# snakers4/mnasnet-pytorch

Hardware: AMD Instinct MI355X
Metric: images/sec MNASNet-1.0 224^2 bf16 train step (higher is better)
Workload: dtype bf16

## Files before the change

include/mnas.h:

```cpp
#ifndef MNAS_H
#define MNAS_H
#include <stdint.h>

#ifdef __cplusplus
extern "C" {
#endif

#define MNAS_OK 0
#define MNAS_EINVAL 10001
#define MNAS_BN_ROWS 8

typedef struct MnasActIn {
    const void*  data;
    const float* scale;
    const float* shift;
} MnasActIn;

typedef struct MnasGradIn {
    const void*  g;
    const void*  y;
    const float* coef;
} MnasGradIn;

int mnas_version(void);
// ... 172 lines not shown
    MnasPostWgrad w1, w2;
} MnasBwdPost;
int mnas_bwd_post(const MnasBwdPost* p, void* stream);

typedef struct MnasBnFrozenDesc {
    const float* gamma;
    const float* beta;
    const float* running_mean;
    const float* running_var;
    float*  bnbuf;
    int32_t C;
    float   eps;
} MnasBnFrozenDesc;
int mnas_bn_frozen_tables(const MnasBnFrozenDesc* descs, int n, void* stream);
int mnas_bn_bwd_finalize_frozen(const float* partial, int nparts, int C, const float* bnbuf, float* dgamma, float* dbeta,
                                float* dbias, int accumulate, void* stream);
typedef struct MnasBwdPostFrozen {
    const float* bn_partial;
    const float* bnbuf;
    float* dgamma;
    float* dbeta;
    double count;
    int32_t bn_nparts, bn_C;
    MnasPostWgrad w1, w2;
    float* dbias;
} MnasBwdPostFrozen;
int mnas_bwd_post_frozen(const MnasBwdPostFrozen* p, void* stream);

int mnas_add_act(const MnasActIn* a, const MnasActIn* b, int64_t rows, int C, void* out_bf16,
                 float* out_nchw_f32, int HW, void* stream);
int mnas_pool_act(const MnasActIn* a, int N, int HW, int C, float* out, void* stream);
int mnas_pool_bwd(const float* gpool, int N, int HW, int C, void* g_bf16, void* stream);
int mnas_nchw_f32_to_nhwc_bf16(const float* src, void* dst, int N, int C, int HW, void* stream);

typedef struct MnasHeadLinear {
    int32_t N, I, O;
    int32_t relu;
    int32_t accumulate;
    float   drop_p;
    uint64_t seed;
    const void* x;
    const void* w;
    const void* b;
    void*       y;
    const void* dz;
    void*       dw;
    void*       db;
    void*       dx;
    const void* relu_mask;
} MnasHeadLinear;
int mnas_head_linear_fwd(const MnasHeadLinear* a, void* stream);
int mnas_head_linear_bwd_w(const MnasHeadLinear* a, void* stream);
int mnas_head_linear_bwd_x(const MnasHeadLinear* a, void* stream);
int mnas_head_dropout_mask(void* out_u8, int64_t n, float p, uint64_t seed, void* stream);
int mnas_head_cross_entropy(const void* logits, const void* target, int N, int C, int64_t ignore_index,
                            void* loss_rows, void* loss, void* dlogits, void* bad_flag, void* stream);

#define MNAS_METERS_MAX_K   4
#define MNAS_METERS_NUM_I64 14
#define MNAS_METERS_NUM_F64 3
typedef struct MnasMeters {
    int64_t steps;
    int64_t samples;
    int64_t loss_samples;
    int64_t nonfinite_steps;
    int64_t correct[MNAS_METERS_MAX_K];
    int64_t last_n;
    int64_t last_loss_n;
    int64_t last_correct[MNAS_METERS_MAX_K];
    double  loss_sum;
    double  last_loss;
    double  last_loss_sum;
} MnasMeters;
int mnas_head_cross_entropy_metrics(const void* logits, const void* target, int N, int C, int64_t ignore_index,
                                    void* loss_rows, void* loss, void* dlogits, void* bad_flag, const int* ks, int nk,
                                    void* rank_rows, MnasMeters* meters, void* stream);
int mnas_head_metrics(const void* logits, const void* target, int N, int C, const int* ks, int nk, const void* loss,
                      void* rank_rows, MnasMeters* meters, void* stream);

int mnas_head_cross_entropy_soft(const void* logits, const void* target_a, const void* target_b, const float* lam,
                                 float label_smoothing, int N, int C, int64_t ignore_index, void* loss_rows, void* loss,
                                 void* dlogits, void* bad_flag, const int* ks, int nk, void* rank_rows, MnasMeters* meters,
                                 void* stream);

#define MNAS_MLABEL_NUM_I64 16
#define MNAS_MLABEL_NUM_F64 9
typedef struct MnasMultiLabelMeters {
    int64_t steps;
    int64_t samples;
    int64_t nonfinite_steps;
    int64_t loss_n;
    int64_t dice_n;
    int64_t f1_n;
    int64_t tp;
    int64_t fp;
    int64_t fn;
    int64_t last_n;
    int64_t last_loss_n;
    int64_t last_dice_n;
    int64_t last_f1_n;
    int64_t last_tp;
    int64_t last_fp;
    int64_t last_fn;
    double  loss_sum;
    double  dice_sum;
    double  f1_sum;
// ... 224 lines not shown
```

mnasnet_pytorch_amd/_lib.py:

```python
from __future__ import annotations

import ctypes as C
import os

import torch

_HERE = os.path.dirname(os.path.abspath(__file__))
ABI_VERSION = 8
LIB_PATH = os.environ.get("MNAS_LIB_PATH") or os.path.join(_HERE, "csrc", "libmnas_hip.so")

c_void_p, c_int, c_float, c_double, c_int64 = C.c_void_p, C.c_int, C.c_float, C.c_double, C.c_int64


class MnasActIn(C.Structure):
    _fields_ = [("data", c_void_p), ("scale", c_void_p), ("shift", c_void_p)]


class MnasGradIn(C.Structure):
    _fields_ = [("g", c_void_p), ("y", c_void_p), ("coef", c_void_p)]


class MnasConvGemm(C.Structure):
    _fields_ = [("mode", C.c_int32), ("N", C.c_int32), ("Hi", C.c_int32), ("Wi", C.c_int32), ("Ci", C.c_int32),
                ("Ho", C.c_int32), ("Wo", C.c_int32), ("Co", C.c_int32), ("kh", C.c_int32), ("kw", C.c_int32),
# ... 236 lines not shown
    kind, k = _SLOT[o.opcode][name]
    return getattr(o, kind)[k]


def op_ints(o):
    return tuple(int(v) for v in o.i[:len(OP_SLOTS[o.opcode][0])])


class MnasHeadLinear(C.Structure):
    _fields_ = [("N", C.c_int32), ("I", C.c_int32), ("O", C.c_int32), ("relu", C.c_int32), ("accumulate", C.c_int32),
                ("drop_p", c_float), ("seed", C.c_uint64), ("x", c_void_p), ("w", c_void_p), ("b", c_void_p),
                ("y", c_void_p), ("dz", c_void_p), ("dw", c_void_p), ("db", c_void_p), ("dx", c_void_p),
                ("relu_mask", c_void_p)]


METERS_MAX_K, METERS_NUM_I64, METERS_NUM_F64 = 4, 14, 3


class MnasMeters(C.Structure):
    _fields_ = [("steps", c_int64), ("samples", c_int64), ("loss_samples", c_int64), ("nonfinite_steps", c_int64),
                ("correct", c_int64 * 4), ("last_n", c_int64), ("last_loss_n", c_int64), ("last_correct", c_int64 * 4),
                ("loss_sum", c_double), ("last_loss", c_double), ("last_loss_sum", c_double)]


MLABEL_NUM_I64, MLABEL_NUM_F64 = 16, 9


class MnasMultiLabelMeters(C.Structure):
    _fields_ = [(n, c_int64) for n in ("steps", "samples", "nonfinite_steps", "loss_n", "dice_n", "f1_n", "tp", "fp", "fn", "last_n",
                                       "last_loss_n", "last_dice_n", "last_f1_n", "last_tp", "last_fp", "last_fn")] + \
               [(n, c_double) for n in ("loss_sum", "dice_sum", "f1_sum", "last_loss", "last_dice", "last_f1", "last_loss_sum",
                                        "last_dice_sum", "last_f1_sum")]


GRADNORM_MAX_PARTS = 1024


class MnasGradStats(C.Structure):
    _fields_ = [("last_norm", c_float), ("last_coef", c_float), ("steps", c_int64), ("clipped_steps", c_int64),
                ("skipped_steps", c_int64)]


class MnasOptExtra(C.Structure):
    _fields_ = [("partial", c_void_p), ("nparts", C.c_int32), ("max_norm", c_float), ("skip_nonfinite", C.c_int32),
                ("ema", c_void_p), ("ema_decay", c_float), ("stats", c_void_p), ("update_stats", C.c_int32)]


SYMBOLS = {
    "mnas_conv_img_parts": (c_int, [c_int] * 11),
    "mnas_stem_parts": (c_int, [c_int, c_int, c_int, c_int, c_int]),
    "mnas_head_linear_fwd": (c_int, [C.POINTER(MnasHeadLinear), c_void_p]),
    "mnas_head_linear_bwd_w": (c_int, [C.POINTER(MnasHeadLinear), c_void_p]),
    "mnas_head_linear_bwd_x": (c_int, [C.POINTER(MnasHeadLinear), c_void_p]),
    "mnas_head_dropout_mask": (c_int, [c_void_p, c_int64, c_float, C.c_uint64, c_void_p]),
    "mnas_head_cross_entropy": (c_int, [c_void_p, c_void_p, c_int, c_int, c_int64, c_void_p, c_void_p, c_void_p, c_void_p,
                                        c_void_p]),
    "mnas_head_cross_entropy_metrics": (c_int, [c_void_p, c_void_p, c_int, c_int, c_int64, c_void_p, c_void_p, c_void_p, c_void_p,
                                                C.POINTER(c_int), c_int, c_void_p, c_void_p, c_void_p]),
    "mnas_head_metrics": (c_int, [c_void_p, c_void_p, c_int, c_int, C.POINTER(c_int), c_int, c_void_p, c_void_p, c_void_p,
                                  c_void_p]),
    "mnas_head_cross_entropy_soft": (c_int, [c_void_p, c_void_p, c_void_p, c_void_p, c_float, c_int, c_int, c_int64, c_void_p,
                                             c_void_p, c_void_p, c_void_p, C.POINTER(c_int), c_int, c_void_p, c_void_p, c_void_p]),
    "mnas_mlabel_scratch_bytes": (c_int64, [c_int]),
    "mnas_mlabel_bce": (c_int, [c_void_p, c_void_p, c_void_p, c_int, c_int, c_int, c_float, c_float, c_void_p, c_void_p, c_void_p,
                                c_void_p, c_int64, c_int64, c_int64, c_void_p]),
    "mnas_mlabel_metrics": (c_int, [c_void_p, c_void_p, c_int, c_int, c_void_p, c_void_p, c_void_p, c_int64, c_int64, c_int64,
                                    c_void_p]),
    "mnas_mlabel_hard_dice": (c_int, [c_void_p, c_void_p, c_int, c_int, c_float, c_int, c_void_p, c_void_p, c_void_p]),
    "mnas_se_scale": (c_int, [C.POINTER(MnasActIn), c_void_p, c_int, c_int, c_int, c_void_p, c_void_p]),
    "mnas_se_bwd_reduce": (c_int, [c_void_p, C.POINTER(MnasActIn), c_void_p, c_int, c_int, c_int, c_void_p, c_void_p, c_void_p]),
    "mnas_se_scratch_bytes": (c_int64, [c_int, c_int, c_int]),
    "mnas_se_bwd_apply": (c_int, [c_void_p, c_void_p, c_void_p, c_int, c_int, c_int, c_void_p, c_void_p, c_void_p, c_void_p, c_void_p]),
    "mnas_se_bwd_apply_cols": (c_int, [c_int, c_int, c_int]),
    "mnas_se_gate": (c_int, [c_void_p, c_int, c_int, c_void_p, c_void_p]),
    "mnas_se_proj_finalize": (c_int, [c_void_p, c_int, c_int, c_int, c_int, c_void_p, c_void_p, c_void_p, c_int, c_void_p, c_void_p]),
    "mnas_stem_dgrad": (c_int, [c_void_p, c_void_p] + [c_int] * 6 + [c_void_p] * 3),
    "mnas_se_fc_supported": (c_int, [c_int, c_int]),
    "mnas_se_fc_fwd": (c_int, [c_void_p] * 5 + [c_int] * 3 + [c_void_p] * 4),
    "mnas_se_fc_bwd": (c_int, [c_void_p] * 5 + [c_int] * 3 + [c_void_p] * 6 + [c_int, c_void_p]),
    "mnas_conv_gemm_gate_ok": (c_int, [c_int, c_int, c_int, c_int]),
    "mnas_graph_create": (c_int, [C.POINTER(MnasOp), c_int, C.POINTER(c_void_p), c_int, C.POINTER(c_void_p), C.POINTER(c_int)]),
    "mnas_graph_launch": (c_int, [c_void_p, c_void_p]),
    "mnas_graph_destroy": (c_int, [c_void_p]),
    "mnas_version": (c_int, []),
    "mnas_arch": (C.c_char_p, []),
    "mnas_workspace_bytes": (c_int64, [c_int, c_int, c_int, c_int]),
    "mnas_conv_gemm": (c_int, [C.POINTER(MnasConvGemm), c_void_p]),
    "mnas_conv_gemm_route": (c_int, [C.POINTER(MnasConvGemm), C.POINTER(c_int)]),
    "mnas_conv_gemm_instance": (c_int, [C.POINTER(MnasConvGemm), C.POINTER(c_int)]),
    "mnas_conv_gemm_tile_pixels": (c_int, [c_int, c_int, c_int]),
    "mnas_conv_gemm_parts": (c_int, [c_int, c_int, c_int, c_int, c_int]),
    "mnas_conv_wgrad": (c_int, [C.POINTER(MnasConvWgrad), c_void_p]),
    "mnas_conv_wgrad_instance": (c_int, [C.POINTER(MnasConvWgrad), C.POINTER(c_int)]),
    "mnas_conv_wgrad_slabs": (c_int, [c_int, c_int, c_int]),
    "mnas_wgrad_finalize": (c_int, [c_void_p, c_int, c_int, c_int, c_int, c_void_p, c_int, c_void_p]),
    "mnas_pw_bwd": (c_int, [C.POINTER(MnasPwBwd), c_void_p]),
    "mnas_pw_bwd_supported": (c_int, [c_int, c_int]),
    "mnas_pw_bwd_forms": (c_int, [c_int, c_int]),
    "mnas_pw_bwd_instance": (c_int, [C.POINTER(MnasPwBwd), C.POINTER(c_int)]),
    "mnas_pw_bwd_tile_pixels": (c_int, [c_int, c_int]),
    "mnas_pw_bwd_slices": (c_int, [c_int, c_int]),
    "mnas_dw_fwd": (c_int, [C.POINTER(MnasDwFwd), c_void_p]),
    "mnas_dw_bwd": (c_int, [C.POINTER(MnasDwBwd), c_void_p]),
    "mnas_dw_rows": (c_int, [c_int, c_int, c_int, c_int, c_int, c_int, c_int]),
    "mnas_dw_geometry": (c_int, [c_int, c_int, c_int, c_int, c_int, c_int, C.POINTER(c_int)]),
    "mnas_dw_wgrad_finalize": (c_int, [c_void_p, c_int, c_int, c_int, c_void_p, c_int, c_void_p]),
# ... 93 lines not shown
```

mnasnet_pytorch_amd/csrc/mnas_elementwise.hip:

```cpp
#include "mnas_common.h"
#ifndef MNAS_FIN_HOIST
#define MNAS_FIN_HOIST 1
#endif

__device__ __forceinline__ double wave_sum_d(double v) {
#pragma unroll
    for (int o = 32; o > 0; o >>= 1) v += __shfl_xor(v, o, 64);
    return v;
}

template <int TPC>
__device__ __forceinline__ void bn_partial_sums(const float* __restrict__ partial, int nparts, int C, int c, double& s1,
                                                double& s2) {
    const int t = threadIdx.x % TPC;
    const float* p1 = partial + (size_t)c * nparts;
    const float* p2 = partial + ((size_t)C + c) * nparts;
    float a1[4] = {0.f, 0.f, 0.f, 0.f}, a2[4] = {0.f, 0.f, 0.f, 0.f};
    for (int p = t; p < nparts; p += 4 * TPC) {
#pragma unroll
        for (int j = 0; j < 4; ++j) {
            const int pj = p + j * TPC;
            const bool ok = pj < nparts;
            a1[j] += ok ? p1[pj] : 0.f;
            a2[j] += ok ? p2[pj] : 0.f;
// ... 565 lines not shown
        } else {
            const int co = i / K, k = i % K;
            const int tap = k / Ci, ci = k % Ci;
            d = grad + ((size_t)co * Ci + ci) * taps + tap;
        }
        if (accumulate) dold = *d;
    }
#endif
    if (i < total) {
        const float* src = partial + i;
        float a[4] = {0.f, 0.f, 0.f, 0.f};
        for (int p = p0 + ty; p < p1; p += 128) {
            float v[16];
#pragma unroll
            for (int j = 0; j < 16; ++j) {
                const int pj = p + 8 * j;
                v[j] = pj < p1 ? src[(size_t)pj * pstride * total] : 0.f;
            }
#pragma unroll
            for (int j = 0; j < 4; ++j) a[j] += (v[j] + v[j + 4]) + (v[j + 8] + v[j + 12]);
        }
        s += (a[0] + a[1]) + (a[2] + a[3]);
    }
    red[ty][tx] = s;
    __syncthreads();
    if (ty == 0 && i < total) {
#pragma unroll
        for (int j = 1; j < 8; ++j) s += red[j][tx];
        if (FOLD) {
            partial[(size_t)p0 * total + i] = s;
            return;
        }
#if MNAS_FIN_HOIST
        *d = dold + s;
#else
        float* d;
        if (DW) {
            const int tap = i / Co, c = i % Co;
            d = grad + (size_t)c * taps + tap;
        } else {
            const int co = i / K, k = i % K;
            const int tap = k / Ci, ci = k % Ci;
            d = grad + ((size_t)co * Ci + ci) * taps + tap;
        }
        *d = (accumulate ? *d : 0.f) + s;
#endif
    }
}
template <bool DW, bool FOLD>
__global__ __launch_bounds__(256) void k_wgrad_finalize(float* __restrict__ partial, int nsplit, int pstride, int Co, int Ci,
                                                         int taps, float* __restrict__ grad, int accumulate) {
    wgrad_finalize_body<DW, FOLD>(partial, nsplit, pstride, Co, Ci, taps, grad, accumulate, blockIdx.x, blockIdx.y);
}

struct PostWg { float* partial; float* grad; int nsplit, Co, Ci, taps, dw, level, nx, ny; };
struct PostArgs {
    const float* bn_partial; float* bnbuf; float* dgamma; float* dbeta; double count;
    int bn_nparts, bn_C, bn_nblk, bn_wide;
    PostWg w1, w2;
};
__device__ __forceinline__ void post_wg(const PostWg& w, int b) {
    const int bx = b % w.nx, by = b / w.nx;
    if (w.level == 2) {
        if (w.dw) wgrad_finalize_body<true, true>(w.partial, w.nsplit, 1, w.Co, w.Ci, w.taps, w.grad, 1, bx, by);
        else wgrad_finalize_body<false, true>(w.partial, w.nsplit, 1, w.Co, w.Ci, w.taps, w.grad, 1, bx, by);
    } else {
        const int ns = w.level == 3 ? (w.nsplit + FIN_SPLITS - 1) / FIN_SPLITS : w.nsplit;
        const int ps = w.level == 3 ? FIN_SPLITS : 1;
        if (w.dw) wgrad_finalize_body<true, false>(w.partial, ns, ps, w.Co, w.Ci, w.taps, w.grad, 1, bx, by);
        else wgrad_finalize_body<false, false>(w.partial, ns, ps, w.Co, w.Ci, w.taps, w.grad, 1, bx, by);
    }
}
__global__ __launch_bounds__(256) void k_bwd_post(PostArgs a) {
    int b = blockIdx.x;
    if (b < a.bn_nblk) {
        if (a.bn_wide) bn_bwd_finalize_body<256>(a.bn_partial, a.bn_nparts, a.bn_C, a.count, a.bnbuf, a.dgamma, a.dbeta, 1, b);
        else bn_bwd_finalize_body<64>(a.bn_partial, a.bn_nparts, a.bn_C, a.count, a.bnbuf, a.dgamma, a.dbeta, 1, b);
        return;
    }
    b -= a.bn_nblk;
    const int n1 = a.w1.level ? a.w1.nx * a.w1.ny : 0;
    if (b < n1) { post_wg(a.w1, b); return; }
    post_wg(a.w2, b - n1);
}
__global__ __launch_bounds__(256) void k_bwd_post_frozen(PostArgs a, float* dbias) {
    int b = blockIdx.x;
    if (b < a.bn_nblk) {
        if (a.bn_wide) bn_bwd_finalize_body<256, true>(a.bn_partial, a.bn_nparts, a.bn_C, a.count, a.bnbuf, a.dgamma, a.dbeta, 1, b, dbias);
        else bn_bwd_finalize_body<64, true>(a.bn_partial, a.bn_nparts, a.bn_C, a.count, a.bnbuf, a.dgamma, a.dbeta, 1, b, dbias);
        return;
    }
    b -= a.bn_nblk;
    const int n1 = a.w1.level ? a.w1.nx * a.w1.ny : 0;
    if (b < n1) { post_wg(a.w1, b); return; }
    post_wg(a.w2, b - n1);
}
static bool post_fill(PostWg* w, const MnasPostWgrad& t) {
    w->level = t.level;
    if (!t.level) { w->nx = w->ny = 0; return true; }
    if (t.level < 1 || t.level > 3 || !t.partial || !t.grad || t.nsplit < 1 || t.Co < 1 || t.Ci < 1 || t.taps < 1) return false;
    if (t.level == 1 && t.nsplit > 2 * FIN_SPLITS) return false;
    w->partial = t.partial; w->grad = t.grad; w->nsplit = t.nsplit; w->Co = t.Co; w->Ci = t.Ci; w->taps = t.taps; w->dw = t.dw;
    const int total = t.dw ? t.Co * t.taps : t.Co * t.Ci * t.taps;
    w->nx = (total + 31) / 32;
    w->ny = t.level == 2 ? (t.nsplit + FIN_SPLITS - 1) / FIN_SPLITS : 1;
    return true;
}
static int post_args(PostArgs* a, const float* bn_partial, const float* bnbuf, float* dgamma, float* dbeta, double count, int bn_nparts,
                     int bn_C, const MnasPostWgrad& w1, const MnasPostWgrad& w2) {
    if (bn_C > 0) {
        if (!bn_partial || !bnbuf || bn_nparts < 1) return -1;
        a->bn_partial = bn_partial; a->bnbuf = const_cast<float*>(bnbuf); a->dgamma = dgamma; a->dbeta = dbeta; a->count = count;
        a->bn_nparts = bn_nparts; a->bn_C = bn_C;
        a->bn_wide = bn_nparts > 256 ? 1 : 0;
        a->bn_nblk = a->bn_wide ? bn_C : (bn_C + 3) / 4;
    }
    if (!post_fill(&a->w1, w1) || !post_fill(&a->w2, w2)) return -1;
    return a->bn_nblk + a->w1.nx * a->w1.ny + a->w2.nx * a->w2.ny;
}
extern "C" int mnas_bwd_post(const MnasBwdPost* p, void* stream) {
    if (!p) return MNAS_EINVAL;
    PostArgs a = {};
    const int blocks = post_args(&a, p->bn_partial, p->bnbuf, p->dgamma, p->dbeta, p->count, p->bn_nparts, p->bn_C, p->w1, p->w2);
    if (blocks < 0) return MNAS_EINVAL;
    if (blocks < 1) return MNAS_OK;
    hipLaunchKernelGGL(k_bwd_post, dim3(blocks), dim3(256), 0, (hipStream_t)stream, a);
    MNAS_CHECK_LAUNCH();
    return MNAS_OK;
}
extern "C" int mnas_bwd_post_frozen(const MnasBwdPostFrozen* p, void* stream) {
    if (!p) return MNAS_EINVAL;
    PostArgs a = {};
    const int blocks = post_args(&a, p->bn_partial, p->bnbuf, p->dgamma, p->dbeta, p->count, p->bn_nparts, p->bn_C, p->w1, p->w2);
    if (blocks < 0) return MNAS_EINVAL;
    if (blocks < 1) return MNAS_OK;
    hipLaunchKernelGGL(k_bwd_post_frozen, dim3(blocks), dim3(256), 0, (hipStream_t)stream, a, p->dbias);
    MNAS_CHECK_LAUNCH();
    return MNAS_OK;
}

template <bool DW>
static int launch_wgrad_finalize(float* partial, int nsplit, int Co, int Ci, int taps, float* grad, int accumulate,
                                 void* stream) {
    if (!partial || !grad || nsplit < 1 || Co < 1 || Ci < 1 || taps < 1) return MNAS_EINVAL;
    const int total = DW ? Co * taps : Co * Ci * taps;
    const int nx = (total + 31) / 32;
    if (nsplit > 2 * FIN_SPLITS) {
        const int ny = (nsplit + FIN_SPLITS - 1) / FIN_SPLITS;
        hipLaunchKernelGGL((k_wgrad_finalize<DW, true>), dim3(nx, ny), dim3(256), 0, (hipStream_t)stream, partial, nsplit, 1,
                           Co, Ci, taps, grad, accumulate);
        hipLaunchKernelGGL((k_wgrad_finalize<DW, false>), dim3(nx, 1), dim3(256), 0, (hipStream_t)stream, partial, ny,
                           FIN_SPLITS, Co, Ci, taps, grad, accumulate);
    } else {
        hipLaunchKernelGGL((k_wgrad_finalize<DW, false>), dim3(nx, 1), dim3(256), 0, (hipStream_t)stream, partial, nsplit, 1,
                           Co, Ci, taps, grad, accumulate);
    }
    MNAS_CHECK_LAUNCH();
    return MNAS_OK;
}
extern "C" int mnas_wgrad_finalize(float* partial, int nsplit, int Co, int Ci, int taps, float* grad,
                                   int accumulate, void* stream) {
    return launch_wgrad_finalize<false>(partial, nsplit, Co, Ci, taps, grad, accumulate, stream);
}
extern "C" int mnas_dw_wgrad_finalize(float* wpartial, int nparts, int C, int k, float* grad, int accumulate,
                                      void* stream) {
    return launch_wgrad_finalize<true>(wpartial, nparts, C, 1, k * k, grad, accumulate, stream);
}

__global__ __launch_bounds__(256) void k_adam(float* __restrict__ p, const float* __restrict__ g, float* __restrict__ m,
                                              float* __restrict__ v, int64_t n, float lr, float b1, float b2, float eps,
                                              float wd, float bc1, float bc2_sqrt, float gscale) {
    for (int64_t i = (int64_t)blockIdx.x * 256 + threadIdx.x; i < n; i += (int64_t)gridDim.x * 256) {
        float gi = g[i] * gscale;
        const float pi = p[i];
        if (wd != 0.f) gi = fmaf(wd, pi, gi);
        const float mi = fmaf(b1, m[i], (1.f - b1) * gi);
        const float vi = fmaf(b2, v[i], (1.f - b2) * gi * gi);
        m[i] = mi;
        v[i] = vi;
        const float denom = sqrtf(vi) / bc2_sqrt + eps;
        p[i] = pi - (lr / bc1) * (mi / denom);
    }
}
__global__ __launch_bounds__(256) void k_rmsprop(float* __restrict__ p, const float* __restrict__ g, float* __restrict__ sq,
                                                 float* __restrict__ buf, int64_t n, float lr, float alpha, float eps, float wd,
                                                 float momentum, float gscale) {
    for (int64_t i = (int64_t)blockIdx.x * 256 + threadIdx.x; i < n; i += (int64_t)gridDim.x * 256) {
        float gi = g[i] * gscale;
        const float pi = p[i];
        if (wd != 0.f) gi = fmaf(wd, pi, gi);
        const float s = fmaf(alpha, sq[i], (1.f - alpha) * gi * gi);
        sq[i] = s;
        const float avg = sqrtf(s) + eps;
        if (momentum > 0.f) {
            const float b = fmaf(momentum, buf[i], gi / avg);
            buf[i] = b;
            p[i] = pi - lr * b;
        } else {
// ... 250 lines not shown
```

mnasnet_pytorch_amd/csrc/mnas_head.hip:

```cpp
#include "mnas_common.h"

__device__ __forceinline__ bool head_keep(unsigned long long seed, unsigned long long idx, unsigned int thresh) {
    unsigned long long z = seed + 0x9E3779B97F4A7C15ull * (idx + 1ull);
    z = (z ^ (z >> 30)) * 0xBF58476D1CE4E5B9ull;
    z = (z ^ (z >> 27)) * 0x94D049BB133111EBull;
    z ^= z >> 31;
    return (unsigned int)(z >> 32) >= thresh;
}

struct HeadGemmArgs {
    int M, N, K;
    const float* A; long long sam, sak;
    const float* B; long long sbk, sbn;
    float* C; long long ldc;
    const float* bias;
    int relu, accumulate;
    int drop_where;
    unsigned int drop_thresh; float drop_scale; unsigned long long seed;
    const float* relu_mask; long long ldm;
    float* rowsum; int rowsum_acc;
};

template <bool VEC>
__global__ __launch_bounds__(512) void k_head_gemm(HeadGemmArgs a) {
    constexpr int BM = 32, BK = 128, LDK = 132, NV = BM * BK / 4 / 512, KW = BK / 8;
    __shared__ __attribute__((aligned(16))) float smem[2 * BM * LDK];
    float* As = smem;
    float* Bs = smem + BM * LDK;
    const int tid = threadIdx.x, lane = tid & 63, wave = tid >> 6;
    const int tx = lane & 7, ty = lane >> 3;
    const int m0 = blockIdx.y * BM, n0 = blockIdx.x * BM;
    float acc[4][4], asum[4];
#pragma unroll
    for (int i = 0; i < 4; ++i) {
        asum[i] = 0.f;
#pragma unroll
        for (int j = 0; j < 4; ++j) acc[i][j] = 0.f;
    }
    const bool a_kfast = a.sak == 1, b_kfast = a.sbk == 1;
    const bool do_rowsum = a.rowsum != nullptr && blockIdx.x == 0;
    float4 ra[NV], rb[NV];
    auto load_op = [&](float4* reg, const float* P, long long sr, long long sk, bool kfast, int r0, int R, int k0, bool drop,
                       long long er, long long ek) {
#pragma unroll
        for (int e = 0; e < NV; ++e) {
            const int q = tid + 512 * e;
            const int rr = kfast ? q / (BK / 4) : (q % (BM / 4)) * 4, kk = kfast ? (q % (BK / 4)) * 4 : q / (BM / 4);
            float v[4] = {0.f, 0.f, 0.f, 0.f};
            const int r = r0 + rr, k = k0 + kk;
            const bool full = kfast ? (r < R && k + 3 < a.K) : (r + 3 < R && k < a.K);
            if (VEC && full) {
                const float4 t = *(const float4*)(P + r * sr + k * sk);
                v[0] = t.x; v[1] = t.y; v[2] = t.z; v[3] = t.w;
            } else {
#pragma unroll
                for (int i = 0; i < 4; ++i) {
                    const int ri = kfast ? r : r + i, ki = kfast ? k + i : k;
                    if (ri < R && ki < a.K) v[i] = P[ri * sr + ki * sk];
                }
            }
            if (drop) {
#pragma unroll
                for (int i = 0; i < 4; ++i) {
                    const int ri = kfast ? r : r + i, ki = kfast ? k + i : k;
                    v[i] = head_keep(a.seed, (unsigned long long)(ri * er + ki * ek), a.drop_thresh) ? v[i] * a.drop_scale : 0.f;
                }
            }
            reg[e] = make_float4(v[0], v[1], v[2], v[3]);
        }
    };
    auto store_op = [&](float* T, const float4* reg, bool kfast) {
#pragma unroll
        for (int e = 0; e < NV; ++e) {
            const int q = tid + 512 * e;
            const int rr = kfast ? q / (BK / 4) : (q % (BM / 4)) * 4, kk = kfast ? (q % (BK / 4)) * 4 : q / (BM / 4);
            if (kfast) {
                *(float4*)(T + rr * LDK + kk) = reg[e];
            } else {
                T[(rr + 0) * LDK + kk] = reg[e].x; T[(rr + 1) * LDK + kk] = reg[e].y;
                T[(rr + 2) * LDK + kk] = reg[e].z; T[(rr + 3) * LDK + kk] = reg[e].w;
            }
        }
    };
    auto load = [&](int k0) {
        load_op(ra, a.A, a.sam, a.sak, a_kfast, m0, a.M, k0, a.drop_where == 1, a.K, 1);
        load_op(rb, a.B, a.sbn, a.sbk, b_kfast, n0, a.N, k0, a.drop_where == 2, 1, a.N);
    };
    load(0);
    for (int k0 = 0; k0 < a.K; k0 += BK) {
        store_op(As, ra, a_kfast);
        store_op(Bs, rb, b_kfast);
        __syncthreads();
        if (k0 + BK < a.K) load(k0 + BK);
// ... 14 lines not shown
                for (int j = 0; j < 4; ++j) {
                    const float br[4] = {bv[j].x, bv[j].y, bv[j].z, bv[j].w};
#pragma unroll
                    for (int c = 0; c < 4; ++c) acc[i][j] = fmaf(ar[c], br[c], acc[i][j]);
                }
            }
        }
        __syncthreads();
    }
    float* part = smem;
#pragma unroll
    for (int i = 0; i < 4; ++i)
#pragma unroll
        for (int j = 0; j < 4; ++j) part[(wave * 32 + ty + 8 * i) * 33 + tx + 8 * j] = acc[i][j];
    __syncthreads();
    float outv[2];
#pragma unroll
    for (int e = 0; e < 2; ++e) {
        const int q = tid + 512 * e, mm = q >> 5, nn = q & 31;
        float v = 0.f;
#pragma unroll
        for (int w = 0; w < 8; ++w) v += part[(w * 32 + mm) * 33 + nn];
        outv[e] = v;
    }
    if (do_rowsum) {
        __syncthreads();
        float* psum = smem;
        if (tx == 0)
#pragma unroll
            for (int i = 0; i < 4; ++i) psum[wave * 32 + ty + 8 * i] = asum[i];
        __syncthreads();
        if (tid < 32 && m0 + tid < a.M) {
            float rs = 0.f;
#pragma unroll
            for (int w = 0; w < 8; ++w) rs += psum[w * 32 + tid];
            a.rowsum[m0 + tid] = a.rowsum_acc ? a.rowsum[m0 + tid] + rs : rs;
        }
    }
#pragma unroll
    for (int e = 0; e < 2; ++e) {
        const int q = tid + 512 * e, mm = q >> 5, nn = q & 31;
        const int m = m0 + mm, n = n0 + nn;
        if (m >= a.M || n >= a.N) continue;
        float v = outv[e];
        if (a.bias) v += a.bias[n];
        if (a.relu) v = fmaxf(v, 0.f);
        if (a.drop_where == 3)
            v = head_keep(a.seed, (unsigned long long)m * a.N + n, a.drop_thresh) ? v * a.drop_scale : 0.f;
        if (a.relu_mask && !(a.relu_mask[m * a.ldm + n] > 0.f)) v = 0.f;
        float* c = a.C + m * a.ldc + n;
        *c = a.accumulate ? *c + v : v;
    }
}

static int head_drop(float p, unsigned int* thresh, float* scale) {
    if (!(p >= 0.f) || p >= 1.f) return MNAS_EINVAL;
    double t = (double)p * 4294967296.0;
    *thresh = t >= 4294967295.0 ? 4294967295u : (unsigned int)t;
    *scale = (float)(1.0 / (1.0 - (double)p));
    return MNAS_OK;
}

static int head_launch(const HeadGemmArgs& a, hipStream_t s) {
    if (a.M < 1 || a.N < 1 || a.K < 1) return MNAS_EINVAL;
    auto vec_ok = [&](const float* P, long long sr, long long sk, int R) {
        const long long lead = sk == 1 ? sr : sk;
        const int extent = sk == 1 ? a.K : R;
        return (sr == 1 || sk == 1) && (lead & 3) == 0 && (extent & 3) == 0 && ((uintptr_t)P & 15) == 0;
    };
    const dim3 grid((a.N + 31) / 32, (a.M + 31) / 32);
    if (vec_ok(a.A, a.sam, a.sak, a.M) && vec_ok(a.B, a.sbn, a.sbk, a.N)) hipLaunchKernelGGL(k_head_gemm<true>, grid, dim3(512), 0, s, a);
    else hipLaunchKernelGGL(k_head_gemm<false>, grid, dim3(512), 0, s, a);
    MNAS_CHECK_LAUNCH();
    return MNAS_OK;
}

extern "C" int mnas_head_linear_fwd(const MnasHeadLinear* c, void* stream) {
    if (!c || !c->x || !c->w || !c->y || c->N < 1 || c->I < 1 || c->O < 1) return MNAS_EINVAL;
    HeadGemmArgs a = {};
    a.M = c->N; a.N = c->O; a.K = c->I;
    a.A = (const float*)c->x; a.sam = c->I; a.sak = 1;
    a.B = (const float*)c->w; a.sbk = 1; a.sbn = c->I;
    a.C = (float*)c->y; a.ldc = c->O;
    a.bias = (const float*)c->b; a.relu = c->relu ? 1 : 0;
    a.seed = c->seed;
    if (c->drop_p > 0.f) {
        if (head_drop(c->drop_p, &a.drop_thresh, &a.drop_scale) != MNAS_OK) return MNAS_EINVAL;
        a.drop_where = 1;
    }
    return head_launch(a, (hipStream_t)stream);
}

extern "C" int mnas_head_linear_bwd_w(const MnasHeadLinear* c, void* stream) {
    if (!c || !c->x || !c->dz || !c->dw || c->N < 1 || c->I < 1 || c->O < 1) return MNAS_EINVAL;
    HeadGemmArgs a = {};
    a.M = c->O; a.N = c->I; a.K = c->N;
    a.A = (const float*)c->dz; a.sam = 1; a.sak = c->O;
    a.B = (const float*)c->x; a.sbk = c->I; a.sbn = 1;
    a.C = (float*)c->dw; a.ldc = c->I; a.accumulate = c->accumulate ? 1 : 0;
    a.rowsum = (float*)c->db; a.rowsum_acc = a.accumulate;
    a.seed = c->seed;
    if (c->drop_p > 0.f) {
        if (head_drop(c->drop_p, &a.drop_thresh, &a.drop_scale) != MNAS_OK) return MNAS_EINVAL;
        a.drop_where = 2;
    }
    return head_launch(a, (hipStream_t)stream);
}

extern "C" int mnas_head_linear_bwd_x(const MnasHeadLinear* c, void* stream) {
    if (!c || !c->dz || !c->w || !c->dx || c->N < 1 || c->I < 1 || c->O < 1) return MNAS_EINVAL;
    HeadGemmArgs a = {};
    a.M = c->N; a.N = c->I; a.K = c->O;
    a.A = (const float*)c->dz; a.sam = c->O; a.sak = 1;
    a.B = (const float*)c->w; a.sbk = c->I; a.sbn = 1;
    a.C = (float*)c->dx; a.ldc = c->I;
    a.relu_mask = (const float*)c->relu_mask; a.ldm = c->I;
    a.seed = c->seed;
    if (c->drop_p > 0.f) {
        if (head_drop(c->drop_p, &a.drop_thresh, &a.drop_scale) != MNAS_OK) return MNAS_EINVAL;
        a.drop_where = 3;
    }
    return head_launch(a, (hipStream_t)stream);
}

__global__ void k_head_mask(unsigned char* out, long long n, unsigned long long seed, unsigned int thresh) {
    const long long i = (long long)blockIdx.x * 256 + threadIdx.x;
    if (i < n) out[i] = head_keep(seed, (unsigned long long)i, thresh) ? 1 : 0;
}
extern "C" int mnas_head_dropout_mask(void* out, int64_t n, float p, uint64_t seed, void* stream) {
    unsigned int thresh; float scale;
    if (!out || n < 1 || head_drop(p, &thresh, &scale) != MNAS_OK) return MNAS_EINVAL;
    hipLaunchKernelGGL(k_head_mask, dim3((unsigned)((n + 255) / 256)), dim3(256), 0, (hipStream_t)stream, (unsigned char*)out,
                       (long long)n, (unsigned long long)seed, thresh);
    MNAS_CHECK_LAUNCH();
    return MNAS_OK;
}

__device__ __forceinline__ float head_wg_reduce(float v, float* red, bool is_max) {
    const int tid = threadIdx.x, lane = tid & 63, wave = tid >> 6;
#pragma unroll
    for (int o = 32; o > 0; o >>= 1) {
        const float w = __shfl_xor(v, o, 64);
        v = is_max ? fmaxf(v, w) : v + w;
    }
    __syncthreads();
    if (lane == 0) red[wave] = v;
    __syncthreads();
    return is_max ? fmaxf(fmaxf(red[0], red[1]), fmaxf(red[2], red[3])) : ((red[0] + red[1]) + red[2]) + red[3];
}

#define HEAD_RANK_WRONG 0x7fffffff

struct HeadKs { int k[MNAS_METERS_MAX_K]; int nk; };

__device__ __forceinline__ int head_wg_reduce_int(int v, int* red) {
    const int tid = threadIdx.x, lane = tid & 63, wave = tid >> 6;
#pragma unroll
    for (int o = 32; o > 0; o >>= 1) v += __shfl_xor(v, o, 64);
    __syncthreads();
    if (lane == 0) red[wave] = v;
    __syncthreads();
    return ((red[0] + red[1]) + red[2]) + red[3];
}

__device__ __forceinline__ void head_meters_update(const int* rank_rows, int N, HeadKs ks, const float* loss, MnasMeters* m, int* redi) {
    int c[MNAS_METERS_MAX_K];
#pragma unroll
    for (int q = 0; q < MNAS_METERS_MAX_K; ++q) c[q] = 0;
    for (int i = threadIdx.x; i < N; i += 256) {
        const int r = rank_rows[i];
#pragma unroll
        for (int q = 0; q < MNAS_METERS_MAX_K; ++q) c[q] += (q < ks.nk && r < ks.k[q]) ? 1 : 0;
    }
#pragma unroll
    for (int q = 0; q < MNAS_METERS_MAX_K; ++q) c[q] = head_wg_reduce_int(c[q], redi);
// ... 262 lines not shown
```

mnasnet_pytorch_amd/head.py:

```python
from __future__ import annotations

import ctypes as C
from typing import List, Optional

import torch
import torch.nn as nn

from . import _lib as L

_MASK64 = (1 << 64) - 1


def _mix(seed: int, a: int, b: int) -> int:
    z = (seed + 0x9E3779B97F4A7C15 * (a + 1) + 0xD1B54A32D192ED03 * (b + 1)) & _MASK64
    z = ((z ^ (z >> 30)) * 0xBF58476D1CE4E5B9) & _MASK64
    z = ((z ^ (z >> 27)) * 0x94D049BB133111EB) & _MASK64
    return z ^ (z >> 31)


class _Layer:
    __slots__ = ("p", "lin", "relu")

    def __init__(self, p, lin):
        self.p, self.lin, self.relu = p, lin, False
# ... 69 lines not shown

    def params(self):
        out = []
        for l in self.layers:
            out.append(l.lin.weight)
            if l.lin.bias is not None:
                out.append(l.lin.bias)
        return out

    def next_seeds(self) -> List[int]:
        self.calls += 1
        return [_mix(self.seed0, self.calls, i) for i in range(len(self.layers))]

    def _check(self, x):
        if x.device.type != "cuda":
            raise RuntimeError("the native head runs on the MI355X only (no CPU path)")
        if x.dim() != 2 or x.shape[1] != self.layers[0].lin.in_features:
            raise ValueError("head input must be (N, %d), got %s" % (self.layers[0].lin.in_features, tuple(x.shape)))

    def _desc(self, l: _Layer, N: int, seed: int) -> L.MnasHeadLinear:
        a = L.MnasHeadLinear()
        a.N, a.I, a.O = N, l.lin.in_features, l.lin.out_features
        a.relu = 1 if l.relu else 0
        a.drop_p = l.p if self.owner.training else 0.0
        a.seed = seed
        a.w = l.lin.weight.data_ptr()
        a.b = L.ptr(l.lin.bias)
        return a

    def forward_layers(self, x, seeds):
        self._check(x)
        x = x.contiguous().float()
        N = x.shape[0]
        us = []
        for l, seed in zip(self.layers, seeds):
            if not (l.lin.weight.is_contiguous() and l.lin.weight.dtype == torch.float32):
                raise RuntimeError("head weights must be contiguous fp32")
            y = torch.empty((N, l.lin.out_features), dtype=torch.float32, device=x.device)
            a = self._desc(l, N, seed)
            a.x, a.y = x.data_ptr(), y.data_ptr()
            L.check(self.lib.mnas_head_linear_fwd(C.byref(a), L.cur_stream()), "head_linear_fwd")
            us.append(x)
            x = y
        return us, x

    def backward_layers(self, us, seeds, dz, grads, accumulate: bool, need_dx: bool = True):
        N = dz.shape[0]
        for i in range(len(self.layers) - 1, -1, -1):
            l = self.layers[i]
            a = self._desc(l, N, seeds[i])
            a.x, a.dz = us[i].data_ptr(), dz.data_ptr()
            a.dw, a.db = grads[i][0].data_ptr(), L.ptr(grads[i][1])
            a.accumulate = 1 if accumulate else 0
            L.check(self.lib.mnas_head_linear_bwd_w(C.byref(a), L.cur_stream()), "head_linear_bwd_w")
            if i == 0 and not need_dx:
                return None
            dx = torch.empty((N, l.lin.in_features), dtype=torch.float32, device=dz.device)
            a.dx = dx.data_ptr()
            a.relu_mask = us[i].data_ptr() if (i > 0 and self.layers[i - 1].relu) else None
            L.check(self.lib.mnas_head_linear_bwd_x(C.byref(a), L.cur_stream()), "head_linear_bwd_x")
            dz = dx
        return dz

    def cross_entropy(self, logits, target, ignore_index=-100, need_grad=True, meters=None):
        N, Cn = logits.shape
        if target.dtype != torch.int64 or target.shape != (N,):
            raise ValueError("target must be int64 of shape (N,)")
        if target.device != logits.device:
            raise RuntimeError("target is on %s, logits on %s (the kernel takes raw device pointers)" % (target.device, logits.device))
        dev = logits.device
        key = (N, dev)
        if key not in self._scratch:
            self._scratch[key] = (torch.empty(N, dtype=torch.float32, device=dev), torch.zeros(1, dtype=torch.int32, device=dev))
        rows, bad = self._scratch[key]
        loss = torch.empty((), dtype=torch.float32, device=dev)
        dl = torch.empty_like(logits) if need_grad else None
        if meters is not None:
            ks, nk, ranks, blk = meters.kernel_args(N, dev)
            L.check(self.lib.mnas_head_cross_entropy_metrics(logits.data_ptr(), target.contiguous().data_ptr(), N, Cn, int(ignore_index),
                                                             rows.data_ptr(), loss.data_ptr(), L.ptr(dl), bad.data_ptr(), ks, nk,
                                                             ranks, blk, L.cur_stream()), "head_cross_entropy_metrics")
            return loss, dl
        L.check(self.lib.mnas_head_cross_entropy(logits.data_ptr(), target.contiguous().data_ptr(), N, Cn, int(ignore_index),
                                                 rows.data_ptr(), loss.data_ptr(), L.ptr(dl), bad.data_ptr(), L.cur_stream()),
                "head_cross_entropy")
        return loss, dl

    def cross_entropy_soft(self, logits, target, label_smoothing=0.0, ignore_index=-100, need_grad=True, meters=None):
        from .losses import soft_cross_entropy, split_target
        a, b, lam = split_target(target)
        if b is None and float(label_smoothing) == 0.0:
            return self.cross_entropy(logits, a, ignore_index, need_grad=need_grad, meters=meters)
        N, dev = logits.shape[0], logits.device
        if b is not None:
            target.check_device(dev)
        key = (N, dev)
        if key not in self._scratch:
            self._scratch[key] = (torch.empty(N, dtype=torch.float32, device=dev), torch.zeros(1, dtype=torch.int32, device=dev))
        rows, bad = self._scratch[key]
        return soft_cross_entropy(logits, a, b, lam, label_smoothing, ignore_index, rows=rows, bad=bad, need_grad=need_grad, meters=meters)

    def bce(self, logits, target, criterion, weights=None, need_grad=True, meters=None, f1_n=None):
        from .losses import bce_with_logits
        N = logits.shape[0]
        if not isinstance(target, torch.Tensor) or target.shape != logits.shape:
            raise ValueError("multi-label target must be of shape (N, C) = %s, got %s"
                             % (tuple(logits.shape), tuple(getattr(target, "shape", ()))))
        target, weights = criterion.prepare(logits, target, weights)
        return bce_with_logits(logits, target, weights, bool(criterion.use_focal_weights), criterion.focus_param,
                               criterion.balance_param, need_grad=need_grad, meters=meters,
                               meter_weights=(N, N, N if f1_n is None else f1_n))

    def check_targets(self):
# ... 33 lines not shown
```

Baseline: 26080.

## Fuse head weight/input grad GEMMs into one launch; add vectorized wgrad finalize

After: 26140, median of 6. About the same (+0.2%).

```diff
diff --git a/include/mnas.h b/include/mnas.h
--- a/include/mnas.h
+++ b/include/mnas.h
@@ -248,6 +248,7 @@
 int mnas_head_linear_fwd(const MnasHeadLinear* a, void* stream);
 int mnas_head_linear_bwd_w(const MnasHeadLinear* a, void* stream);
 int mnas_head_linear_bwd_x(const MnasHeadLinear* a, void* stream);
+int mnas_head_linear_bwd(const MnasHeadLinear* a, void* stream);
 int mnas_head_dropout_mask(void* out_u8, int64_t n, float p, uint64_t seed, void* stream);
 int mnas_head_cross_entropy(const void* logits, const void* target, int N, int C, int64_t ignore_index,
                             void* loss_rows, void* loss, void* dlogits, void* bad_flag, void* stream);
diff --git a/mnasnet_pytorch_amd/_lib.py b/mnasnet_pytorch_amd/_lib.py
--- a/mnasnet_pytorch_amd/_lib.py
+++ b/mnasnet_pytorch_amd/_lib.py
@@ -312,6 +312,7 @@
     "mnas_head_linear_fwd": (c_int, [C.POINTER(MnasHeadLinear), c_void_p]),
     "mnas_head_linear_bwd_w": (c_int, [C.POINTER(MnasHeadLinear), c_void_p]),
     "mnas_head_linear_bwd_x": (c_int, [C.POINTER(MnasHeadLinear), c_void_p]),
+    "mnas_head_linear_bwd": (c_int, [C.POINTER(MnasHeadLinear), c_void_p]),
     "mnas_head_dropout_mask": (c_int, [c_void_p, c_int64, c_float, C.c_uint64, c_void_p]),
     "mnas_head_cross_entropy": (c_int, [c_void_p, c_void_p, c_int, c_int, c_int64, c_void_p, c_void_p, c_void_p, c_void_p,
                                         c_void_p]),
diff --git a/mnasnet_pytorch_amd/csrc/mnas_elementwise.hip b/mnasnet_pytorch_amd/csrc/mnas_elementwise.hip
--- a/mnasnet_pytorch_amd/csrc/mnas_elementwise.hip
+++ b/mnasnet_pytorch_amd/csrc/mnas_elementwise.hip
@@ -641,6 +641,66 @@
                                                          int taps, float* __restrict__ grad, int accumulate) {
     wgrad_finalize_body<DW, FOLD>(partial, nsplit, pstride, Co, Ci, taps, grad, accumulate, blockIdx.x, blockIdx.y);
 }
+template <bool DW, bool FOLD>
+__global__ __launch_bounds__(256) void k_wgrad_finalize_wide(float* __restrict__ partial, int nsplit, int pstride, int Co, int Ci,
+                                                              int taps, float* __restrict__ grad, int accumulate) {
+    const int bx = blockIdx.x, by = blockIdx.y;
+    __shared__ __attribute__((aligned(16))) float red[8][128];
+    const int K = taps * Ci;
+    const int total = DW ? Co * taps : Co * K;
+    const int tid = threadIdx.x, tx = tid & 31, ty = tid >> 5;
+    const int i = bx * 128 + 4 * tx;
+    const int io = bx * 128 + tid;
+    const int p0 = FOLD ? by * FIN_SPLITS : 0, p1 = FOLD ? min(nsplit, p0 + FIN_SPLITS) : nsplit;
+    float* d = nullptr;
+    float dold = 0.f;
+    if (!FOLD && tid < 128 && io < total) {
+        if (DW) {
+            const int tap = io / Co, c = io % Co;
+            d = grad + (size_t)c * taps + tap;
+        } else {
+            const int co = io / K, k = io % K;
+            const int tap = k / Ci, ci = k % Ci;
+            d = grad + ((size_t)co * Ci + ci) * taps + tap;
+        }
+        if (accumulate) dold = *d;
+    }
+    float s[4] = {0.f, 0.f, 0.f, 0.f};
+    if (i < total) {
+        const float* src = partial + i;
+        float a[4][4];
+#pragma unroll
+        for (int j = 0; j < 4; ++j)
+#pragma unroll
+            for (int c = 0; c < 4; ++c) a[j][c] = 0.f;
+        for (int p = p0 + ty; p < p1; p += 128) {
+            float4 v[16];
+#pragma unroll
+            for (int j = 0; j < 16; ++j) {
+                const int pj = p + 8 * j;
+                v[j] = pj < p1 ? *(const float4*)(src + (size_t)pj * pstride * total) : make_float4(0.f, 0.f, 0.f, 0.f);
+            }
+#pragma unroll
+            for (int j = 0; j < 4; ++j) {
+                a[j][0] += (v[j].x + v[j + 4].x) + (v[j + 8].x + v[j + 12].x);
+                a[j][1] += (v[j].y + v[j + 4].y) + (v[j + 8].y + v[j + 12].y);
+                a[j][2] += (v[j].z + v[j + 4].z) + (v[j + 8].z + v[j + 12].z);
+                a[j][3] += (v[j].w + v[j + 4].w) + (v[j + 8].w + v[j + 12].w);
+            }
+        }
+#pragma unroll
+        for (int c = 0; c < 4; ++c) s[c] += (a[0][c] + a[1][c]) + (a[2][c] + a[3][c]);
+    }
+    *(float4*)&red[ty][4 * tx] = make_float4(s[0], s[1], s[2], s[3]);
+    __syncthreads();
+    if (tid < 128 && io < total) {
+        float r = red[0][tid];
+#pragma unroll
+        for (int j = 1; j < 8; ++j) r += red[j][tid];
+        if (FOLD) partial[(size_t)p0 * total + io] = r;
+        else *d = dold + r;
+    }
+}
 
 struct PostWg { float* partial; float* grad; int nsplit, Co, Ci, taps, dw, level, nx, ny; };
 struct PostArgs {
@@ -733,6 +793,21 @@
                                  void* stream) {
     if (!partial || !grad || nsplit < 1 || Co < 1 || Ci < 1 || taps < 1) return MNAS_EINVAL;
     const int total = DW ? Co * taps : Co * Ci * taps;
+    if ((total & 3) == 0 && ((uintptr_t)partial & 15) == 0) {
+        const int nx = (total + 127) / 128;
+        if (nsplit > 2 * FIN_SPLITS) {
+            const int ny = (nsplit + FIN_SPLITS - 1) / FIN_SPLITS;
+            hipLaunchKernelGGL((k_wgrad_finalize_wide<DW, true>), dim3(nx, ny), dim3(256), 0, (hipStream_t)stream, partial, nsplit, 1,
+                               Co, Ci, taps, grad, accumulate);
+            hipLaunchKernelGGL((k_wgrad_finalize_wide<DW, false>), dim3(nx, 1), dim3(256), 0, (hipStream_t)stream, partial, ny,
+                               FIN_SPLITS, Co, Ci, taps, grad, accumulate);
+        } else {
+            hipLaunchKernelGGL((k_wgrad_finalize_wide<DW, false>), dim3(nx, 1), dim3(256), 0, (hipStream_t)stream, partial, nsplit, 1,
+                               Co, Ci, taps, grad, accumulate);
+        }
+        MNAS_CHECK_LAUNCH();
+        return MNAS_OK;
+    }
     const int nx = (total + 31) / 32;
     if (nsplit > 2 * FIN_SPLITS) {
         const int ny = (nsplit + FIN_SPLITS - 1) / FIN_SPLITS;
diff --git a/mnasnet_pytorch_amd/csrc/mnas_head.hip b/mnasnet_pytorch_amd/csrc/mnas_head.hip
--- a/mnasnet_pytorch_amd/csrc/mnas_head.hip
+++ b/mnasnet_pytorch_amd/csrc/mnas_head.hip
@@ -21,15 +21,16 @@
     float* rowsum; int rowsum_acc;
 };
 
+constexpr int HEAD_SMEM = 2 * 32 * 132;
 template <bool VEC>
-__global__ __launch_bounds__(512) void k_head_gemm(HeadGemmArgs a) {
+__device__ __forceinline__ void head_gemm_body(const HeadGemmArgs& a, const int bx, const int by, float* smem) {
     constexpr int BM = 32, BK = 128, LDK = 132, NV = BM * BK / 4 / 512, KW = BK / 8;
-    __shared__ __attribute__((aligned(16))) float smem[2 * BM * LDK];
+    static_assert(HEAD_SMEM == 2 * BM * LDK, "operand tiles");
     float* As = smem;
     float* Bs = smem + BM * LDK;
     const int tid = threadIdx.x, lane = tid & 63, wave = tid >> 6;
     const int tx = lane & 7, ty = lane >> 3;
-    const int m0 = blockIdx.y * BM, n0 = blockIdx.x * BM;
+    const int m0 = by * BM, n0 = bx * BM;
     float acc[4][4], asum[4];
 #pragma unroll
     for (int i = 0; i < 4; ++i) {
@@ -38,7 +39,7 @@
         for (int j = 0; j < 4; ++j) acc[i][j] = 0.f;
     }
     const bool a_kfast = a.sak == 1, b_kfast = a.sbk == 1;
-    const bool do_rowsum = a.rowsum != nullptr && blockIdx.x == 0;
+    const bool do_rowsum = a.rowsum != nullptr && bx == 0;
     float4 ra[NV], rb[NV];
     auto load_op = [&](float4* reg, const float* P, long long sr, long long sk, bool kfast, int r0, int R, int k0, bool drop,
                        long long er, long long ek) {
@@ -159,6 +160,20 @@
         *c = a.accumulate ? *c + v : v;
     }
 }
+template <bool VEC>
+__global__ __launch_bounds__(512) void k_head_gemm(HeadGemmArgs a) {
+    __shared__ __attribute__((aligned(16))) float smem[HEAD_SMEM];
+    head_gemm_body<VEC>(a, blockIdx.x, blockIdx.y, smem);
+}
+
+struct HeadGemmPair { HeadGemmArgs p0, p1; int nb0, gx0, gx1; };
+template <bool VEC0, bool VEC1>
+__global__ __launch_bounds__(512) void k_head_gemm_pair(HeadGemmPair p) {
+    __shared__ __attribute__((aligned(16))) float smem[HEAD_SMEM];
+    const int b = blockIdx.x;
+    if (b < p.nb0) head_gemm_body<VEC0>(p.p0, b % p.gx0, b / p.gx0, smem);
+    else head_gemm_body<VEC1>(p.p1, (b - p.nb0) % p.gx1, (b - p.nb0) / p.gx1, smem);
+}
 
 static int head_drop(float p, unsigned int* thresh, float* scale) {
     if (!(p >= 0.f) || p >= 1.f) return MNAS_EINVAL;
@@ -168,16 +183,38 @@
     return MNAS_OK;
 }
 
-static int head_launch(const HeadGemmArgs& a, hipStream_t s) {
-    if (a.M < 1 || a.N < 1 || a.K < 1) return MNAS_EINVAL;
+static bool head_vec_ok(const HeadGemmArgs& a) {
     auto vec_ok = [&](const float* P, long long sr, long long sk, int R) {
         const long long lead = sk == 1 ? sr : sk;
         const int extent = sk == 1 ? a.K : R;
         return (sr == 1 || sk == 1) && (lead & 3) == 0 && (extent & 3) == 0 && ((uintptr_t)P & 15) == 0;
     };
+    return vec_ok(a.A, a.sam, a.sak, a.M) && vec_ok(a.B, a.sbn, a.sbk, a.N);
+}
+
+static int head_launch(const HeadGemmArgs& a, hipStream_t s) {
+    if (a.M < 1 || a.N < 1 || a.K < 1) return MNAS_EINVAL;
     const dim3 grid((a.N + 31) / 32, (a.M + 31) / 32);
-    if (vec_ok(a.A, a.sam, a.sak, a.M) && vec_ok(a.B, a.sbn, a.sbk, a.N)) hipLaunchKernelGGL(k_head_gemm<true>, grid, dim3(512), 0, s, a);
+    if (head_vec_ok(a)) hipLaunchKernelGGL(k_head_gemm<true>, grid, dim3(512), 0, s, a);
     else hipLaunchKernelGGL(k_head_gemm<false>, grid, dim3(512), 0, s, a);
+    MNAS_CHECK_LAUNCH();
+    return MNAS_OK;
+}
+
+static int head_launch_pair(const HeadGemmArgs& a0, const HeadGemmArgs& a1, hipStream_t s) {
+    if (a0.M < 1 || a0.N < 1 || a0.K < 1 || a1.M < 1 || a1.N < 1 || a1.K < 1) return MNAS_EINVAL;
+    HeadGemmPair p;
+    p.p0 = a0; p.p1 = a1;
+    p.gx0 = (a0.N + 31) / 32; p.gx1 = (a1.N + 31) / 32;
+    const long long nb0 = (long long)p.gx0 * ((a0.M + 31) / 32), nb1 = (long long)p.gx1 * ((a1.M + 31) / 32);
+    if (nb0 + nb1 > 0x7fffffffll) return MNAS_EINVAL;
+    p.nb0 = (int)nb0;
+    const dim3 grid((unsigned)(nb0 + nb1));
+    const bool v0 = head_vec_ok(a0), v1 = head_vec_ok(a1);
+    if (v0 && v1) hipLaunchKernelGGL((k_head_gemm_pair<true, true>), grid, dim3(512), 0, s, p);
+    else if (v0) hipLaunchKernelGGL((k_head_gemm_pair<true, false>), grid, dim3(512), 0, s, p);
+    else if (v1) hipLaunchKernelGGL((k_head_gemm_pair<false, true>), grid, dim3(512), 0, s, p);
+    else hipLaunchKernelGGL((k_head_gemm_pair<false, false>), grid, dim3(512), 0, s, p);
     MNAS_CHECK_LAUNCH();
     return MNAS_OK;
 }
@@ -198,7 +235,7 @@
     return head_launch(a, (hipStream_t)stream);
 }
 
-extern "C" int mnas_head_linear_bwd_w(const MnasHeadLinear* c, void* stream) {
+static int head_fill_bwd_w(const MnasHeadLinear* c, HeadGemmArgs* out) {
     if (!c || !c->x || !c->dz || !c->dw || c->N < 1 || c->I < 1 || c->O < 1) return MNAS_EINVAL;
     HeadGemmArgs a = {};
     a.M = c->O; a.N = c->I; a.K = c->N;
@@ -211,10 +248,16 @@
         if (head_drop(c->drop_p, &a.drop_thresh, &a.drop_scale) != MNAS_OK) return MNAS_EINVAL;
         a.drop_where = 2;
     }
+    *out = a;
+    return MNAS_OK;
+}
+extern "C" int mnas_head_linear_bwd_w(const MnasHeadLinear* c, void* stream) {
+    HeadGemmArgs a;
+    if (head_fill_bwd_w(c, &a) != MNAS_OK) return MNAS_EINVAL;
     return head_launch(a, (hipStream_t)stream);
 }
 
-extern "C" int mnas_head_linear_bwd_x(const MnasHeadLinear* c, void* stream) {
+static int head_fill_bwd_x(const MnasHeadLinear* c, HeadGemmArgs* out) {
     if (!c || !c->dz || !c->w || !c->dx || c->N < 1 || c->I < 1 || c->O < 1) return MNAS_EINVAL;
     HeadGemmArgs a = {};
     a.M = c->N; a.N = c->I; a.K = c->O;
@@ -227,7 +270,19 @@
         if (head_drop(c->drop_p, &a.drop_thresh, &a.drop_scale) != MNAS_OK) return MNAS_EINVAL;
         a.drop_where = 3;
     }
+    *out = a;
+    return MNAS_OK;
+}
+extern "C" int mnas_head_linear_bwd_x(const MnasHeadLinear* c, void* stream) {
+    HeadGemmArgs a;
+    if (head_fill_bwd_x(c, &a) != MNAS_OK) return MNAS_EINVAL;
     return head_launch(a, (hipStream_t)stream);
+}
+
+extern "C" int mnas_head_linear_bwd(const MnasHeadLinear* c, void* stream) {
+    HeadGemmArgs aw, ax;
+    if (head_fill_bwd_w(c, &aw) != MNAS_OK || head_fill_bwd_x(c, &ax) != MNAS_OK) return MNAS_EINVAL;
+    return head_launch_pair(aw, ax, (hipStream_t)stream);
 }
 
 __global__ void k_head_mask(unsigned char* out, long long n, unsigned long long seed, unsigned int thresh) {
diff --git a/mnasnet_pytorch_amd/head.py b/mnasnet_pytorch_amd/head.py
--- a/mnasnet_pytorch_amd/head.py
+++ b/mnasnet_pytorch_amd/head.py
@@ -145,13 +145,13 @@
             a.x, a.dz = us[i].data_ptr(), dz.data_ptr()
             a.dw, a.db = grads[i][0].data_ptr(), L.ptr(grads[i][1])
             a.accumulate = 1 if accumulate else 0
-            L.check(self.lib.mnas_head_linear_bwd_w(C.byref(a), L.cur_stream()), "head_linear_bwd_w")
             if i == 0 and not need_dx:
+                L.check(self.lib.mnas_head_linear_bwd_w(C.byref(a), L.cur_stream()), "head_linear_bwd_w")
                 return None
             dx = torch.empty((N, l.lin.in_features), dtype=torch.float32, device=dz.device)
             a.dx = dx.data_ptr()
             a.relu_mask = us[i].data_ptr() if (i > 0 and self.layers[i - 1].relu) else None
-            L.check(self.lib.mnas_head_linear_bwd_x(C.byref(a), L.cur_stream()), "head_linear_bwd_x")
+            L.check(self.lib.mnas_head_linear_bwd(C.byref(a), L.cur_stream()), "head_linear_bwd")
             dz = dx
         return dz
 
```
